# Dhole/collaborative_filtering

Measured on AMD Instinct MI355X. Metric: user-subgraph eigendecomps/sec + predicted ratings/sec, 1M users avg deg 100, higher is better.
Workload: dtype f32 (eigen) / f64 (predict)

## Files before the change

collaborative_filtering_amd/_native.py:

```python
from __future__ import annotations

import ctypes
import os
from ctypes import POINTER, c_char_p, c_double, c_float, c_int, c_int32, c_uint32, c_uint64, c_void_p

_HERE = os.path.dirname(os.path.abspath(__file__))
LIB_PATH = os.environ.get("CF_MI355X_LIB") or os.path.join(_HERE, "libcf_mi355x.so")
HOST_LIB_PATH = os.path.join(_HERE, "libcf_host.so")

CF_OK = 0
CF_EINVAL = -1
CF_ERANGE = -4
CF_SVD_MAX_NV = 256
CF_ALS_MAX_D = 64
CF_TOPN_MAX_N = 1024
CF_SIGS_OWN = 0
CF_SIGS_COMPAT = 1
CF_MAX_K = 192
CF_SPILL_MAX_K = 5000
CF_EIGEN_TRIDIAG = 0
CF_EIGEN_JACOBI = 1
CF_GRAPH_DENSE = 0
CF_GRAPH_CSR = 1
CF_FILTER_CHEBY = 0
CF_FILTER_BINOMIAL = 1

SIGNATURES = {
    "cf_version": (c_int, []),
    "cf_device_count": (c_int, []),
    "cf_create": (c_int, [c_int, POINTER(c_void_p)]),
    "cf_destroy": (None, [c_void_p]),
    "cf_release_workspaces": (c_int, [c_void_p]),
    "cf_last_error": (c_char_p, [c_void_p]),
    "cf_set_jacobi": (c_int, [c_void_p, c_float, c_int]),
    "cf_set_eigen_refine": (c_int, [c_void_p, c_int, c_float, c_float]),
    "cf_set_eigen_split": (c_int, [c_void_p, c_int]),
    "cf_debug_split_schedule": (c_int, [c_int, c_int, POINTER(c_int), POINTER(c_int), POINTER(c_int), POINTER(c_int)]),
    "cf_set_step_masks": (c_int, [c_void_p, c_int]),
    "cf_set_local_wlim": (c_int, [c_void_p, c_int]),
    "cf_debug_predict_nmax": (c_int, [c_int]),
    "cf_set_knn2_topk": (c_int, [c_void_p, c_uint32]),
    "cf_set_eigen_method": (c_int, [c_void_p, c_int]),
    "cf_debug_stats": (c_int, [c_void_p, c_int, c_void_p]),
    "cf_eigen_bucket_timing": (c_int, [c_void_p, c_int, c_void_p]),
    "cf_eigen_bucket_timing_split": (c_int, [c_void_p, c_int, c_void_p, c_void_p]),
    "cf_debug_phases": (c_int, [c_void_p, c_int, c_void_p]),
    "cf_debug_spill": (c_int, [c_void_p, c_int, c_void_p]),
    "cf_debug_tri": (c_int, [c_void_p, c_int, c_void_p]),
    "cf_item_graph_upload": (c_int, [c_void_p, c_uint32, c_void_p, c_void_p, c_void_p]),
    "cf_item_graph_upload_dense": (c_int, [c_void_p, c_uint32, c_void_p, c_int]),
    "cf_item_graph_device": (c_void_p, [c_void_p, POINTER(c_uint32)]),
    "cf_set_graph_layout": (c_int, [c_void_p, c_int]),
    "cf_graph_info": (c_int, [c_void_p, c_void_p, c_void_p, c_void_p]),
    "cf_item_cosine_edges": (c_int, [c_void_p, c_uint32, c_uint32, c_void_p, c_void_p, c_void_p, c_float, c_int, c_int,
                                     c_void_p, c_void_p, c_void_p, c_uint64, c_void_p]),
    "cf_plan_create": (c_int, [c_void_p, c_uint32, c_void_p, POINTER(c_void_p)]),
    "cf_plan_destroy": (None, [c_void_p]),
    "cf_evec_slots": (c_uint64, [c_uint32]),
    "cf_evec_offsets": (c_uint64, [c_uint32, c_void_p, c_void_p]),
    "cf_eigen_batch": (c_int, [c_void_p, c_uint32, c_void_p, c_void_p, c_void_p, c_void_p, c_void_p,
                               c_void_p, c_void_p]),
    "cf_eigen_run": (c_int, [c_void_p, c_void_p, c_void_p, c_void_p, c_void_p, c_void_p, c_void_p,
                             c_void_p, c_void_p, c_void_p]),
    "cf_predict_precomp": (c_int, [c_void_p, c_uint32, c_void_p, c_void_p, c_void_p, c_void_p, c_void_p,
                                   c_void_p, c_void_p, c_void_p, c_uint64, c_int, c_void_p, c_void_p,
                                   c_void_p]),
    "cf_predict_precomp_sel": (c_int, [c_void_p, c_uint32, c_void_p, c_void_p, c_void_p, c_void_p, c_void_p,
                                       c_void_p, c_void_p, c_void_p, c_uint64, c_int, c_void_p, c_void_p,
                                       c_void_p, c_void_p]),
# ... 169 lines not shown
```

collaborative_filtering_amd/api.py:

```python
from __future__ import annotations

from ctypes import byref, c_double, c_float, c_int, c_uint32, c_void_p
from dataclasses import dataclass

import numpy as np

from . import _native
from ._native import CF_ERANGE, CF_FILTER_BINOMIAL, CF_FILTER_CHEBY, CF_SIGS_COMPAT, CF_SIGS_OWN, NativeError, ptr


def _check(lib, ctx, rc, what):
    if rc != _native.CF_OK:
        msg = lib.cf_last_error(ctx)
        raise NativeError(f"{what} failed ({rc}): {msg.decode() if msg else ''}")


def evec_offsets(item_off: np.ndarray) -> tuple[np.ndarray, int]:
    k = np.diff(item_off.astype(np.int64))
    slots = k * np.maximum(k, 2)
    off = np.zeros(len(k), dtype=np.uint64)
    if len(k):
        off[1:] = np.cumsum(slots)[:-1]
    return off, int(slots.sum())

# ... 149 lines not shown
            self.lib.cf_destroy(self.h)
            self.h = None

    def release_workspaces(self):
        self._chk(self.lib.cf_release_workspaces(self.h), "cf_release_workspaces")

    def __enter__(self):
        return self

    def __exit__(self, *exc):
        self.close()

    def __del__(self):
        try:
            self.close()
        except Exception:
            pass

    def _chk(self, rc, what):
        _check(self.lib, self.h, rc, what)

    def set_eigen_method(self, method: str = "jacobi"):
        code = {"tridiag": _native.CF_EIGEN_TRIDIAG, "jacobi": _native.CF_EIGEN_JACOBI}[method]
        self._chk(self.lib.cf_set_eigen_method(self.h, code), "cf_set_eigen_method")

    def set_jacobi(self, tol_scale: float = 1.0, max_sweeps: int = 30):
        self._chk(self.lib.cf_set_jacobi(self.h, tol_scale, max_sweeps), "cf_set_jacobi")

    def set_eigen_refine(self, enable: bool = True, stop_rel: float = 1e-3, delta: float = 1e-2):
        self._chk(self.lib.cf_set_eigen_refine(self.h, int(enable), stop_rel, delta), "cf_set_eigen_refine")

    def set_eigen_split(self, enable=True):
        self._chk(self.lib.cf_set_eigen_split(self.h, int(enable)), "cf_set_eigen_split")

    def set_local_wlim(self, bisect: bool = True):
        self._chk(self.lib.cf_set_local_wlim(self.h, int(bisect)), "cf_set_local_wlim")

    def set_step_masks(self, enable: bool = True):
        self._chk(self.lib.cf_set_step_masks(self.h, int(enable)), "cf_set_step_masks")

    def debug_stats(self, enable: bool = True, read: bool = False):
        out = np.zeros(8, dtype=np.uint64) if read else None
        self._chk(self.lib.cf_debug_stats(self.h, int(enable), ptr(out)), "cf_debug_stats")
        if read:
            n = max(int(out[1]), 1)
            return {"sweeps_mean": int(out[0]) / n, "users": int(out[1]), "sweeps_max": int(out[2]),
                    "capped": int(out[3]), "assembly_cyc_per_user": int(out[4]) / n,
                    "jacobi_cyc_per_user": int(out[5]) / n, "epilogue_cyc_per_user": int(out[6]) / n,
                    "jacobi_cyc_per_step": int(out[5]) / max(int(out[7]), 1)}
        return None

    def eigen_bucket_timing(self, enable: bool = True, read: bool = False, sweeps: bool = False):
        out = np.zeros(13, dtype=np.float32) if read else None
        sw = np.zeros(13, dtype=np.float32) if read else None
        self._chk(self.lib.cf_eigen_bucket_timing_split(self.h, int(enable), ptr(out), ptr(sw)),
                  "cf_eigen_bucket_timing_split")
        return (out, sw) if sweeps else out

    def debug_spill(self, enable: bool = True, read: bool = False):
        out = np.zeros(8, dtype=np.uint64) if read else None
        self._chk(self.lib.cf_debug_spill(self.h, int(enable), ptr(out)), "cf_debug_spill")
        if read:
            n = max(int(out[0]), 1)
            names = ["assembly", "tridiag", "accumulate", "ql", "ql_gen"]
            r = {f"{nm}_cyc_per_user": int(out[i + 1]) / n for i, nm in enumerate(names)}
            r.update(users=int(out[0]), ql_iters_per_user=int(out[6]) / n, output_cyc_per_user=int(out[7]) / n)
# ... 790 lines not shown
```

collaborative_filtering_amd/csrc/cf_eigen.hip:

```cpp

#include "cf_eigen_common.h"

namespace {
using namespace cf_eig;

template <int EMAX, bool NARROW = false>
struct EigenGeom {
    static constexpr int NR = 16 * EMAX;
    static constexpr int NC = NARROW ? 188 : NR;
    static constexpr int E2 = NR / (2 * kGroup);
    static constexpr int LD16 = NR + ((16 - NR) % 64 + 64) % 64;
    static constexpr int LD = (NC * LD16 + 9 * NR <= 40960 - 4) ? LD16 : NR + 8;
    static constexpr int NT = (NR > 128) ? 1024 : 512;
    static constexpr int WPE = EMAX <= 5 ? 6 : 4;

    static constexpr size_t bytes() {
        return sizeof(float) * (size_t)NC * LD
               + sizeof(uint32_t) * NR
               + sizeof(float) * NR * 5
               + sizeof(int) * NR
               + sizeof(int) * 4;
    }
};
static_assert(EigenGeom<12, true>::LD % 64 == 16, "narrow bucket-12 layout must be conflict-free");
// ... 531 lines not shown
            int steps = 0;
            for (int L = 0; ((n + (1 << L) - 1) >> L) >= 2; ++L) steps += (((n + (1 << L) - 1) >> L) + 1) >> 1;
            atomicAdd(&a.stats[7], (unsigned long long)((sweep + 1) * steps));
        }
    }
}

template <int EMAX, bool NARROW = false, bool RESUME = false>
int launch_bucket_k(cf_ctx* ctx, const EigenArgs& args, uint32_t count, hipStream_t stream) {
    using G = EigenGeom<EMAX, NARROW>;
    const size_t lds = G::bytes();
    static_assert(G::bytes() <= 163840, "eigen bucket exceeds 160 KiB LDS");
    static bool configured = false;
    if (!configured) {
        CF_HIP_CHECK(ctx, hipFuncSetAttribute((const void*)eigen_kernel<EMAX, NARROW, RESUME>,
                                              hipFuncAttributeMaxDynamicSharedMemorySize, (int)lds));
        configured = true;
    }
    hipLaunchKernelGGL((eigen_kernel<EMAX, NARROW, RESUME>), dim3(count), dim3(G::NT), lds, stream, args);
    CF_HIP_CHECK(ctx, hipGetLastError());
    return CF_OK;
}

template <int EMAX, bool NARROW = false>
int launch_bucket(cf_ctx* ctx, const EigenArgs& args, uint32_t count, hipStream_t stream, uint32_t kmax = 0) {
    if constexpr (EMAX >= kSplitEmaxLow) {
        bool handled = false, finished = false;
        CF_TRY(launch_split_sweeps(ctx, args, EMAX, count, kmax, stream, &handled, &finished));
        if (handled && finished) return CF_OK;
        if (handled) {
            if (ctx->split_mid_ev) {
                CF_HIP_CHECK(ctx, hipEventRecord(ctx->split_mid_ev, stream));
                ctx->split_mid_recorded = true;
            }
            return launch_bucket_k<EMAX, NARROW, true>(ctx, args, count, stream);
        }
    }
    return launch_bucket_k<EMAX, NARROW, false>(ctx, args, count, stream);
}

int launch_bucket12_layout(cf_ctx* ctx, const EigenArgs& args, uint32_t count, uint32_t kmax, hipStream_t stream) {
    static const bool narrow_on = [] {
        const char* e = getenv("CF_EIGEN_NARROW");
        return !(e && e[0] == '0');
    }();
    if (narrow_on && kmax <= (uint32_t)EigenGeom<12, true>::NC) return launch_bucket<12, true>(ctx, args, count, stream, kmax);
    return launch_bucket<12>(ctx, args, count, stream, kmax);
}

int launch_bucket12(cf_ctx* ctx, const cf_plan* plan, const EigenArgs& args, uint32_t count, uint32_t kmax,
                    hipStream_t stream) {
    if (plan && args.mode == kUser && kmax > (uint32_t)kSplitKmax12 && count > 1) {
        auto k_at = [&](uint32_t j) {
            const uint32_t u = plan->h_order[args.first + j];
            return (uint32_t)(plan->h_item_off[u + 1] - plan->h_item_off[u]);
        };
        uint32_t lo = 0, hi = count;
        while (lo < hi) {
            const uint32_t mid = (lo + hi) / 2;
            if (k_at(mid) > (uint32_t)kSplitKmax12) lo = mid + 1;
            else hi = mid;
        }
        if (lo > 0 && lo < count) {
            CF_TRY(launch_bucket12_layout(ctx, args, lo, kmax, stream));
            EigenArgs rest = args;
            rest.first += lo;
// ... 315 lines not shown
```

collaborative_filtering_amd/csrc/cf_eigen_common.h:

```cpp
#pragma once

#include "cf_internal.h"

namespace cf_eig {

constexpr int kGroup = 8;
#ifndef CF_EIGEN_SIGROT2
#define CF_EIGEN_SIGROT2 256.0f
#endif
constexpr float kSigRot2 = CF_EIGEN_SIGROT2;

using f2 = __attribute__((ext_vector_type(2))) float;
using f4 = __attribute__((ext_vector_type(4))) float;
__device__ __forceinline__ f2 lds_ld(const f2* p) {
    return *(const volatile __attribute__((address_space(3))) f2*)(p);
}
__device__ __forceinline__ void lds_st(f2* p, f2 v) {
#if defined(CF_EIGEN_FUSED_ST) && CF_EIGEN_FUSED_ST
    *p = v;
#else
    *(volatile __attribute__((address_space(3))) f2*)(p) = v;
#endif
}

// ... 39 lines not shown
    const uint32_t* pair_user;
    const uint64_t* test_off;
    const uint32_t* test_user;
    const float* test_rating;
    float* wlim;
    const int* only_flag;
    uint64_t* cmask_out;
    uint64_t cmask_words;
    uint64_t* cmask_fp;
    uint32_t cmask_users;
    const uint8_t* solved;
    int skip_spill;
    int skip_emax_min;
};

__device__ __forceinline__ float test_rating(const EigenArgs& a, uint32_t movie, uint32_t user) {
    uint64_t lo = a.test_off[movie];
    const uint64_t end = a.test_off[movie + 1];
    uint64_t hi = end;
    while (lo < hi) {
        const uint64_t mid = (lo + hi) >> 1;
        if (a.test_user[mid] < user) lo = mid + 1;
        else hi = mid;
    }
    return (lo < end && a.test_user[lo] == user) ? a.test_rating[lo] : 0.0f;
}

constexpr int kSplitEmaxMin = 9;
constexpr int kSplitEmaxLow = 5;
constexpr int kSplitKmax12 = 180;
int launch_split_sweeps(cf_ctx* ctx, const EigenArgs& a, int emax, uint32_t count, uint32_t kmax, hipStream_t stream,
                        bool* handled, bool* finished);

}
```

collaborative_filtering_amd/csrc/cf_eigen_split.hip:

```cpp

#include <array>
#include <mutex>

#include "cf_eigen_common.h"

namespace cf_eig {
namespace {

constexpr int kMaxLev = 9;
constexpr uint32_t kNone = 0xFFFFFFFFu;
constexpr uint32_t kRoleActive = 1u << 31;
constexpr uint32_t kTrWrite = 1u << 31;
constexpr uint32_t kTrRead = 1u << 30;
constexpr int kTrFLShift = 16;

constexpr int split_ld(int nr) {
    int ld = nr;
    while (ld % 64 != 16 && ld % 64 != 48) ++ld;
    return ld;
}

constexpr int split_upc(int emax) { return emax >= 9 ? 2 : 3; }

template <int EMAX>
// ... 1020 lines not shown
        const int RBo = (NS * LD) / LDO;
        for (int i0 = 0; i0 < k; i0 += RBo) {
            const int rb = min(RBo, k - i0);
            for (int idx = tid; idx < rb * k; idx += NT) {
                const int r = idx / k, c = idx - r * k;
                tile[r * LDO + c] = hb[(size_t)(i0 + r) * k + c];
            }
            __syncthreads();
            for (int idx = tid; idx < rb * lim; idx += NT) {
                const int r = idx / lim, cc = idx - r * lim;
                float v = 0.0f;
                if (cc < k) {
                    const int jj = s_map[cc];
                    v = tile[r * LDO + jj] * s_s[jj];
                }
                hb[(size_t)(i0 + r) * lim + cc] = v;
            }
            __syncthreads();
        }
    }
    if (a.stats && tid == 0) {
        const unsigned long long t3 = __builtin_amdgcn_s_memtime();
        atomicAdd(&a.stats[0], (unsigned long long)(sweep + 1));
        atomicAdd(&a.stats[1], 1ull);
        atomicMax(&a.stats[2], (unsigned long long)(sweep + 1));
        if (sweep >= a.max_sweeps) atomicAdd(&a.stats[3], 1ull);
        atomicAdd(&a.stats[4], s_stamp[1] - s_stamp[0]);
        atomicAdd(&a.stats[5], s_stamp[2] - s_stamp[1]);
        if (FINISH) atomicAdd(&a.stats[6], t3 - s_stamp[2]);
        atomicAdd(&a.stats[7], (unsigned long long)((sweep + 1) * steps_sweep));
    }
}

template <int EMAX, bool FINISH>
int launch_split_kernel(cf_ctx* ctx, const EigenArgs& a, uint32_t count, hipStream_t stream) {
    using G = SplitGeom<EMAX>;
    static bool configured = false;
    if (!configured) {
        CF_HIP_CHECK(ctx, hipFuncSetAttribute((const void*)split_sweep_kernel<EMAX, FINISH>,
                                              hipFuncAttributeMaxDynamicSharedMemorySize, (int)G::bytes()));
        configured = true;
    }
    hipLaunchKernelGGL((split_sweep_kernel<EMAX, FINISH>), dim3(count), dim3(G::NT), G::bytes(), stream, a,
                       (const uint32_t*)ctx->d_split_sched[EMAX]);
    CF_HIP_CHECK(ctx, hipGetLastError());
    return CF_OK;
}

template <int EMAX>
int launch_emax_split(cf_ctx* ctx, const EigenArgs& a, uint32_t count, uint32_t kmax, hipStream_t stream,
                      bool* handled, bool* finished) {
    int ok_hi = 0;
    const std::vector<uint32_t>& tab = host_table<EMAX>(&ok_hi);
    if ((int)kmax > ok_hi) return CF_OK;
    if (!ctx->d_split_sched[EMAX]) {
        void* p = nullptr;
        CF_TRY(cf_malloc_evict(ctx, &p, tab.size() * sizeof(uint32_t), "split sweep schedule"));
        ctx->d_split_sched[EMAX] = static_cast<uint32_t*>(p);
        CF_HIP_CHECK(ctx, hipMemcpy(p, tab.data(), tab.size() * sizeof(uint32_t), hipMemcpyHostToDevice));
    }
    if (ctx->split_finish < 0) {
        const char* e = getenv("CF_EIGEN_SPLIT_FINISH");
        ctx->split_finish = !e ? 2 : (e[0] == '1') ? 1 : 0;
    }
    if (ctx->split_finish == 1 || (ctx->split_finish == 2 && EMAX <= 8)) {
        CF_TRY((launch_split_kernel<EMAX, true>(ctx, a, count, stream)));
// ... 1 lines not shown
    } else {
        CF_TRY((launch_split_kernel<EMAX, false>(ctx, a, count, stream)));
    }
    *handled = true;
    return CF_OK;
}

}

int launch_split_sweeps(cf_ctx* ctx, const EigenArgs& a, int emax, uint32_t count, uint32_t kmax, hipStream_t stream,
                        bool* handled, bool* finished) {
    *handled = false;
    *finished = false;
    if (a.mode != kUser || emax < kSplitEmaxLow || emax > 12 || count == 0) return CF_OK;
    if (ctx->eigen_split < 0) {
        const char* e = getenv("CF_EIGEN_SPLIT");
        ctx->eigen_split = e ? atoi(e) : 1;
    }
    const int emin = ctx->eigen_split == 1 ? kSplitEmaxMin : ctx->eigen_split;
    if (!ctx->eigen_split || emax < emin) return CF_OK;
    switch (emax) {
        case 5: return launch_emax_split<5>(ctx, a, count, kmax, stream, handled, finished);
        case 6: return launch_emax_split<6>(ctx, a, count, kmax, stream, handled, finished);
        case 7: return launch_emax_split<7>(ctx, a, count, kmax, stream, handled, finished);
        case 8: return launch_emax_split<8>(ctx, a, count, kmax, stream, handled, finished);
        case 9: return launch_emax_split<9>(ctx, a, count, kmax, stream, handled, finished);
        case 10: return launch_emax_split<10>(ctx, a, count, kmax, stream, handled, finished);
        case 11: return launch_emax_split<11>(ctx, a, count, kmax, stream, handled, finished);
        case 12: return launch_emax_split<12>(ctx, a, count, kmax, stream, handled, finished);
        default: return CF_OK;
    }
}

}

using namespace cf_eig;

extern "C" int cf_set_eigen_split(cf_ctx* ctx, int enable) {
    if (!ctx) return CF_EINVAL;
    if (enable < 0 || (enable > 1 && (enable < kSplitEmaxLow || enable > 12))) return CF_EINVAL;
    ctx->eigen_split = enable;
    return CF_OK;
}

namespace {
template <int EMAX>
void geom_of(int* ng, int* ns, int* klo, int* khi) {
    *ng = SplitGeom<EMAX>::NG;
    *ns = SplitGeom<EMAX>::NS;
    *klo = SplitGeom<EMAX>::KLO;
    *khi = SplitGeom<EMAX>::KHI;
}
}

extern "C" int cf_debug_split_schedule(int emax, int k, int* steps, int* levels, int* max_groups, int* max_slots) {
    int NG, NS, klo, khi;
    switch (emax) {
        case 5: geom_of<5>(&NG, &NS, &klo, &khi); break;
        case 6: geom_of<6>(&NG, &NS, &klo, &khi); break;
        case 7: geom_of<7>(&NG, &NS, &klo, &khi); break;
        case 8: geom_of<8>(&NG, &NS, &klo, &khi); break;
        case 9: geom_of<9>(&NG, &NS, &klo, &khi); break;
        case 10: geom_of<10>(&NG, &NS, &klo, &khi); break;
        case 11: geom_of<11>(&NG, &NS, &klo, &khi); break;
        case 12: geom_of<12>(&NG, &NS, &klo, &khi); break;
        default: return CF_ERANGE;
    }
    if (k < klo || k > khi) return CF_ERANGE;
    Schedule S;
// ... 10 lines not shown
```

collaborative_filtering_amd/csrc/cf_internal.h:

```cpp
#pragma once

#include <hip/hip_runtime.h>

#include <algorithm>
#include <cstdint>
#include <string>
#include <vector>

#include "cf_abi.h"

struct GraphRow {
    const float* dense;
    const uint32_t* col;
    const float* w;
    uint32_t len;
    __device__ __forceinline__ float operator[](uint32_t b) const {
        if (dense) return dense[b];
        uint32_t lo = 0, hi = len;
        while (lo < hi) {
            const uint32_t mid = (lo + hi) >> 1;
            if (col[mid] < b) lo = mid + 1;
            else hi = mid;
        }
        return (lo < len && col[lo] == b) ? w[lo] : 0.0f;
// ... 70 lines not shown
    void* d_tri = nullptr;
    size_t tri_bytes = 0;
    int eigen_method = CF_EIGEN_JACOBI;
    bool tri_debug = false;
    hipEvent_t knn_ev[3] = {nullptr, nullptr, nullptr};
    int knn_path = 0;
    unsigned int* d_knn_acc = nullptr;
    void* d_knn_part = nullptr;
    size_t knn_part_bytes = 0;
    uint32_t knn_chunk_users = 0;
    uint32_t knn2_topk = 0;
    int knn_chunks = 0;
    void* d_prep = nullptr;
    size_t prep_bytes = 0;
    hipEvent_t prep_ev[2] = {nullptr, nullptr};
    static constexpr int kAuxStreams = 2;
    hipStream_t aux_stream[kAuxStreams] = {};
    hipEvent_t aux_event[kAuxStreams + 1] = {};
    static constexpr int kBucketRuns = 16;
    bool bucket_timing = false;
    hipEvent_t bucket_ev[kBucketRuns][13][3] = {};
    bool bucket_recorded[kBucketRuns][13] = {};
    bool bucket_mid[kBucketRuns][13] = {};
    hipEvent_t split_mid_ev = nullptr;
    bool split_mid_recorded = false;
    int bucket_run = 0;
    hipStream_t step_stream[2] = {};
    hipEvent_t step_bucket_ev[16] = {};
    hipEvent_t step_sync_ev[4] = {};
    hipEvent_t step_time_ev[3] = {};
    uint32_t* d_split_sched[13] = {};
    int eigen_split = -1;
    int split_finish = -1;
    float filter_ms = 0.0f;
    uint64_t filter_nnz = 0;
    void* d_als = nullptr;
    size_t als_bytes = 0;
    float sgd_reduce_ms[2] = {0.0f, 0.0f};
    float svdpp_reduce_ms[3] = {0.0f, 0.0f, 0.0f};
    uint32_t topn_block = 0;
};

constexpr int kSpillBucket = -1;

struct cf_bucket {
    int emax = 0;

    uint32_t count = 0;
    uint32_t first = 0;
    uint32_t kmax = 0;
};

struct cf_tri_chunk {
    int emax;
    uint32_t first;
    uint32_t count;
    uint32_t kmax;
    uint32_t group;
};
struct cf_tri_group {
    uint32_t first;
    uint32_t count;
    uint32_t kmax;
};

struct cf_plan {
// ... 178 lines not shown
```

collaborative_filtering_amd/csrc/cf_pack.hip:

```cpp

#include <algorithm>
#include <thread>
#include <vector>

#include "cf_internal.h"

namespace {

constexpr int kScanThreads = 1024;

__global__ void __launch_bounds__(kScanThreads) pack_offsets_kernel(uint32_t n_users, const uint64_t* item_off,
                                                                    const int32_t* m, uint64_t* packed_off) {
    __shared__ uint64_t s_sum[kScanThreads];
    const uint32_t t = threadIdx.x;
    const uint32_t chunk = (n_users + kScanThreads - 1) / kScanThreads;
    const uint32_t u0 = min(n_users, t * chunk), u1 = min(n_users, u0 + chunk);
    uint64_t s = 0;
    for (uint32_t u = u0; u < u1; ++u) s += (item_off[u + 1] - item_off[u]) * (uint64_t)max(m[u], 0);
    s_sum[t] = s;
    __syncthreads();
    for (int d = 1; d < kScanThreads; d <<= 1) {
        const uint64_t v = t >= (uint32_t)d ? s_sum[t - d] : 0;
        __syncthreads();
        s_sum[t] += v;
        __syncthreads();
    }
    uint64_t run = s_sum[t] - s;
    for (uint32_t u = u0; u < u1; ++u) {
        packed_off[u] = run;
        run += (item_off[u + 1] - item_off[u]) * (uint64_t)max(m[u], 0);
    }
    if (t == kScanThreads - 1) packed_off[n_users] = s_sum[t];
}

__global__ void __launch_bounds__(256) pack_copy_kernel(uint32_t n_users, const uint64_t* item_off, const int32_t* m,
                                                        const uint64_t* evec_off, const float* evecs,
                                                        const uint64_t* packed_off, float* packed) {
    for (uint32_t u = blockIdx.x; u < n_users; u += gridDim.x) {
        const uint64_t n = (item_off[u + 1] - item_off[u]) * (uint64_t)max(m[u], 0);
        const float* src = evecs + evec_off[u];
        float* dst = packed + packed_off[u];
        const uint64_t mis_s = ((uintptr_t)src >> 2) & 3, mis_d = ((uintptr_t)dst >> 2) & 3;
        if (mis_s == mis_d) {
            const uint64_t head = min<uint64_t>(n, (4 - mis_s) & 3);
            for (uint64_t i = threadIdx.x; i < head; i += blockDim.x) dst[i] = src[i];
            const uint64_t nv = (n - head) / 4;
            const float4* s4 = reinterpret_cast<const float4*>(src + head);
            float4* d4 = reinterpret_cast<float4*>(dst + head);
            for (uint64_t i = threadIdx.x; i < nv; i += blockDim.x) d4[i] = s4[i];
            for (uint64_t i = head + nv * 4 + threadIdx.x; i < n; i += blockDim.x) dst[i] = src[i];
        } else {
            for (uint64_t i = threadIdx.x; i < n; i += blockDim.x) dst[i] = src[i];
        }
    }
}

void cost_split(uint32_t n_users, const uint64_t* item_off, int n_parts, uint32_t* split) {
    std::vector<double> cum(n_users + 1, 0.0);
    for (uint32_t u = 0; u < n_users; ++u) {
        const double k = (double)(item_off[u + 1] - item_off[u]);
        cum[u + 1] = cum[u] + k * k * k;
    }
    split[0] = 0;
    for (int p = 1; p < n_parts; ++p) {
        const double target = cum[n_users] * (double)p / (double)n_parts;
// ... 38 lines not shown
            for (uint32_t u = 0; u <= nu; ++u) off[u] = item_off[u0 + u] - e0;
            for (uint32_t u = 0; u < nu; ++u) eoff[u] = evec_off[u0 + u] - lo;
            const bool compat = sig_mode == CF_SIGS_COMPAT;
            rcs[d] = sel(ctxs[d], nu, off.data(), items + e0, ratings + e0, m + u0, evals + e0,
                                            eoff.data(), evecs + lo, compat ? sigtab : sigtab + e0,
                                            compat ? sigtab_len : ne, sig_mode, row_sel ? row_sel + e0 : nullptr,
                                            mse + e0, kk + e0, pred ? pred + e0 : nullptr);
        });
    for (auto& t : pool) t.join();
    for (int d = 0; d < n_dev; ++d)
        if (rcs[d] != CF_OK)
            return cf_set_error(root, rcs[d], "device part " + std::to_string(d) + ": " + ctxs[d]->last_error);
    (void)hipSetDevice(root->device);
    return CF_OK;
}

}

extern "C" {

int cf_cost_split(uint32_t n_users, const uint64_t* item_off, int n_parts, uint32_t* split) {
    if (!item_off || !split || n_parts <= 0) return CF_EINVAL;
    cost_split(n_users, item_off, n_parts, split);
    return CF_OK;
}

int cf_pack_eigen_run(cf_ctx* ctx, uint32_t n_users, const uint64_t* d_item_off, const int32_t* d_m,
                      const uint64_t* d_evec_off, const float* d_evecs, uint64_t* d_packed_off, float* d_packed,
                      void* stream) {
    if (!ctx || !d_item_off || !d_m || !d_packed_off) return cf_set_error(ctx, CF_EINVAL, "cf_pack_eigen_run: null");
    if (d_packed && (!d_evec_off || !d_evecs)) return cf_set_error(ctx, CF_EINVAL, "cf_pack_eigen_run: null evecs");
    CF_TRY(set_device(ctx));
    hipStream_t st = (hipStream_t)stream;
    hipLaunchKernelGGL(pack_offsets_kernel, dim3(1), dim3(kScanThreads), 0, st, n_users, d_item_off, d_m,
                       d_packed_off);
    CF_HIP_CHECK(ctx, hipGetLastError());
    if (d_packed && n_users) {
        const uint32_t blocks = std::min<uint32_t>(n_users, 65536u);
        hipLaunchKernelGGL(pack_copy_kernel, dim3(blocks), dim3(256), 0, st, n_users, d_item_off, d_m, d_evec_off,
                           d_evecs, (const uint64_t*)d_packed_off, d_packed);
        CF_HIP_CHECK(ctx, hipGetLastError());
    }
    return CF_OK;
}

struct multi_part {
    cf_ctx* ctx = nullptr;
    uint32_t u0 = 0, n = 0;
    uint64_t e0 = 0, ne = 0;
    uint64_t packed = 0;
    DevBuf off, items, eoff, m, sig, eval, evec, poff, pack;
    hipStream_t stream = nullptr;
    int rc = CF_OK;
};

static int multi_run_part(multi_part& p, const uint64_t* item_off, const uint32_t* items) {
    cf_ctx* ctx = p.ctx;
    CF_TRY(set_device(ctx));
    CF_HIP_CHECK(ctx, hipStreamCreateWithFlags(&p.stream, hipStreamNonBlocking));
    std::vector<uint64_t> off(p.n + 1), eoff(std::max<uint32_t>(p.n, 1));
    for (uint32_t u = 0; u <= p.n; ++u) off[u] = item_off[p.u0 + u] - p.e0;
    const uint64_t n_evec = cf_evec_offsets(p.n, off.data(), eoff.data());
    for (uint64_t e = 0; e < p.ne; ++e)
        if (items[p.e0 + e] >= ctx->n_items) return cf_set_error(ctx, CF_EINVAL, "item index outside the graph");
    cf_plan* plan = nullptr;
    CF_TRY(cf_plan_create(ctx, p.n, off.data(), &plan));
    int rc = dev_alloc(ctx, p.off, sizeof(uint64_t) * (p.n + 1));
    if (rc == CF_OK) rc = dev_alloc(ctx, p.items, sizeof(uint32_t) * p.ne);
    if (rc == CF_OK) rc = dev_alloc(ctx, p.eoff, sizeof(uint64_t) * eoff.size());
// ... 168 lines not shown
```

include/cf_abi.h:

```cpp
#ifndef CF_ABI_H
#define CF_ABI_H

#include <stddef.h>
#include <stdint.h>

#ifdef __cplusplus
extern "C" {
#endif

#define CF_OK 0
#define CF_EINVAL (-1)
#define CF_ENOMEM (-2)
#define CF_EHIP (-3)
#define CF_ERANGE (-4)
#define CF_ESTATE (-5)

#define CF_MAX_K 192
#define CF_SPILL_MAX_K 5000

typedef struct cf_ctx cf_ctx;
typedef struct cf_plan cf_plan;

int cf_version(void);
int cf_device_count(void);
int cf_create(int device, cf_ctx** out);
void cf_destroy(cf_ctx* ctx);
int cf_release_workspaces(cf_ctx* ctx);
const char* cf_last_error(const cf_ctx* ctx);
#define CF_EIGEN_TRIDIAG 0
#define CF_EIGEN_JACOBI 1
int cf_set_eigen_method(cf_ctx* ctx, int method);
int cf_set_jacobi(cf_ctx* ctx, float tol_scale, int max_sweeps);
int cf_set_eigen_refine(cf_ctx* ctx, int enable, float stop_rel, float delta);
int cf_set_eigen_split(cf_ctx* ctx, int enable);
int cf_debug_split_schedule(int emax, int k, int* steps, int* levels, int* max_groups, int* max_slots);
int cf_set_step_masks(cf_ctx* ctx, int enable);
int cf_set_local_wlim(cf_ctx* ctx, int bisect);
int cf_debug_stats(cf_ctx* ctx, int enable, uint64_t* out8);
int cf_debug_spill(cf_ctx* ctx, int enable, uint64_t* out8);
int cf_debug_tri(cf_ctx* ctx, int enable, uint64_t* out8);
int cf_debug_phases(cf_ctx* ctx, int enable, uint64_t* out16);
int cf_debug_predict_nmax(int lmax);
int cf_eigen_bucket_timing(cf_ctx* ctx, int enable, float* ms13);
int cf_eigen_bucket_timing_split(cf_ctx* ctx, int enable, float* ms13, float* sweeps_ms13);

#define CF_GRAPH_DENSE 0
#define CF_GRAPH_CSR 1
int cf_set_graph_layout(cf_ctx* ctx, int layout);
int cf_graph_info(const cf_ctx* ctx, int* layout, uint32_t* n_items, uint64_t* nnz);
int cf_item_graph_upload(cf_ctx* ctx, uint32_t n_items, const uint64_t* row_ptr,
                         const uint32_t* col, const float* w);
int cf_item_graph_upload_dense(cf_ctx* ctx, uint32_t n_items, const float* w_dense,
                               int on_device);
const float* cf_item_graph_device(const cf_ctx* ctx, uint32_t* n_items);

int cf_plan_create(cf_ctx* ctx, uint32_t n_users, const uint64_t* item_off, cf_plan** out);
void cf_plan_destroy(cf_plan* plan);
uint64_t cf_evec_slots(uint32_t k);
uint64_t cf_evec_offsets(uint32_t n_users, const uint64_t* item_off, uint64_t* evec_off);

int cf_eigen_batch(cf_ctx* ctx, uint32_t n_users, const uint64_t* item_off,
                   const uint32_t* items, const uint64_t* evec_off, int32_t* m_out,
                   float* sigs, float* evals, float* evecs);
int cf_eigen_run(cf_ctx* ctx, const cf_plan* plan, const uint64_t* d_item_off,
                 const uint32_t* d_items, const uint64_t* d_evec_off, int32_t* d_m,
                 float* d_sigs, float* d_evals, float* d_evecs, void* stream);

// ... 240 lines not shown
```

Before: 330,800.

## Add dedicated split-finish eigen kernel and multi-block pack offset scan

Adds a separate finish kernel for eigen buckets 9-12 after split sweeps. It does the refinement correction with MFMA, fp64 norm and sign normalisation, rank sort, limit count and transpose in a smaller-LDS workgroup sized so two fit per CU. It replaces the resumed full eigen kernel epilogue, which should improve occupancy for the tail phase. Separately, the single-block pack offset scan becomes a three-kernel multi-block decoupled scan, to remove a serial bottleneck over 1M users.

Result: no change. 332,600 (median of 6 runs) (+0.6%).

```diff
diff --git a/collaborative_filtering_amd/_native.py b/collaborative_filtering_amd/_native.py
--- a/collaborative_filtering_amd/_native.py
+++ b/collaborative_filtering_amd/_native.py
@@ -35,6 +35,7 @@
     "cf_set_jacobi": (c_int, [c_void_p, c_float, c_int]),
     "cf_set_eigen_refine": (c_int, [c_void_p, c_int, c_float, c_float]),
     "cf_set_eigen_split": (c_int, [c_void_p, c_int]),
+    "cf_set_eigen_finish": (c_int, [c_void_p, c_int]),
     "cf_debug_split_schedule": (c_int, [c_int, c_int, POINTER(c_int), POINTER(c_int), POINTER(c_int), POINTER(c_int)]),
     "cf_set_step_masks": (c_int, [c_void_p, c_int]),
     "cf_set_local_wlim": (c_int, [c_void_p, c_int]),
diff --git a/collaborative_filtering_amd/api.py b/collaborative_filtering_amd/api.py
--- a/collaborative_filtering_amd/api.py
+++ b/collaborative_filtering_amd/api.py
@@ -205,6 +205,9 @@
 
     def set_eigen_split(self, enable=True):
         self._chk(self.lib.cf_set_eigen_split(self.h, int(enable)), "cf_set_eigen_split")
+
+    def set_eigen_finish(self, mode=1):
+        self._chk(self.lib.cf_set_eigen_finish(self.h, int(mode)), "cf_set_eigen_finish")
 
     def set_local_wlim(self, bisect: bool = True):
         self._chk(self.lib.cf_set_local_wlim(self.h, int(bisect)), "cf_set_local_wlim")
diff --git a/collaborative_filtering_amd/csrc/cf_eigen.hip b/collaborative_filtering_amd/csrc/cf_eigen.hip
--- a/collaborative_filtering_amd/csrc/cf_eigen.hip
+++ b/collaborative_filtering_amd/csrc/cf_eigen.hip
@@ -587,6 +587,11 @@
             if (ctx->split_mid_ev) {
                 CF_HIP_CHECK(ctx, hipEventRecord(ctx->split_mid_ev, stream));
                 ctx->split_mid_recorded = true;
+            }
+            if constexpr (EMAX >= kSplitEmaxMin) {
+                bool launched = false;
+                CF_TRY(launch_split_finish(ctx, args, EMAX, count, stream, &launched));
+                if (launched) return CF_OK;
             }
             return launch_bucket_k<EMAX, NARROW, true>(ctx, args, count, stream);
         }
diff --git a/collaborative_filtering_amd/csrc/cf_eigen_common.h b/collaborative_filtering_amd/csrc/cf_eigen_common.h
--- a/collaborative_filtering_amd/csrc/cf_eigen_common.h
+++ b/collaborative_filtering_amd/csrc/cf_eigen_common.h
@@ -95,4 +95,6 @@
 int launch_split_sweeps(cf_ctx* ctx, const EigenArgs& a, int emax, uint32_t count, uint32_t kmax, hipStream_t stream,
                         bool* handled, bool* finished);
 
+int launch_split_finish(cf_ctx* ctx, const EigenArgs& a, int emax, uint32_t count, hipStream_t stream, bool* launched);
+
 }
diff --git a/collaborative_filtering_amd/csrc/cf_eigen_split.hip b/collaborative_filtering_amd/csrc/cf_eigen_split.hip
--- a/collaborative_filtering_amd/csrc/cf_eigen_split.hip
+++ b/collaborative_filtering_amd/csrc/cf_eigen_split.hip
@@ -1076,6 +1076,380 @@
     }
 }
 
+template <int EMAX>
+struct FinishGeom {
+    using S = SplitGeom<EMAX>;
+    static constexpr int NR = S::NR, KLO = S::KLO, KHI = S::KHI;
+    static constexpr int NW = 4, NT = 64 * NW, NG = NT / kGroup;
+    static constexpr int TJ = (EMAX + NW - 1) / NW;
+    static constexpr int CPG = (KHI + NG - 1) / NG;
+    static constexpr int SMALL = 4 * NR * 4 + 16;
+    static constexpr int STATIC = 256;
+    static constexpr int AREA = ((81920 - STATIC - SMALL) / 4) & ~3;
+    static constexpr int RB1x = ((AREA / KHI - 4) / 16) * 16;
+    static constexpr int RB1 = RB1x < NR ? RB1x : NR, LDR1 = RB1 + 4;
+    static constexpr int RB3 = 32, LDR3 = RB3 + 4;
+    static constexpr int DOFF = (KHI * LDR3 + 3) & ~3;
+    static constexpr int TB = 32, TBW = 2 * TB * (TB + 1);
+    static constexpr size_t bytes() { return (size_t)AREA * 4 + SMALL; }
+    static_assert(EMAX >= 9 && EMAX <= 12, "buckets 9-12");
+    static_assert(KLO > 16 * (EMAX - 1), "every k of the bucket has EMAX column tiles");
+    static_assert(KHI <= NT, "a thread per eigenvalue in the lim count");
+    static_assert(RB1 >= 16 && RB1 % 16 == 0 && NR * LDR1 <= AREA, "F row block (NR columns: unguarded reads)");
+    static_assert(NR * LDR3 <= AREA, "update row block (NR columns: unguarded reads)");
+    static_assert(RB3 % 16 == 0 && LDR3 % 8 == 4 && DOFF + 4 * CPG * NT <= AREA, "update row block, fp64 partials");
+    static_assert(NW * TBW <= AREA, "flip blocks");
+    static_assert(16 * (KHI + 1) <= AREA && NR <= AREA, "output row block, sigs");
+    static_assert((bytes() + STATIC) * 2 <= 163840, "two finish workgroups share a CU's LDS");
+};
+
+template <int EMAX>
+__global__ __launch_bounds__(FinishGeom<EMAX>::NT, 2) void split_finish_kernel(EigenArgs a) {
+    using G = FinishGeom<EMAX>;
+    constexpr int NR = G::NR, NW = G::NW, NT = G::NT, NG = G::NG, TJ = G::TJ, CPG = G::CPG;
+    constexpr int RB1 = G::RB1, LDR1 = G::LDR1, RB3 = G::RB3, LDR3 = G::LDR3;
+    extern __shared__ float smem[];
+    float* tile = smem;
+    float* s_mu = tile + G::AREA;
+    float* s_dev = s_mu + NR;
+    float* s_s = s_dev + NR;
+    int* s_perm = reinterpret_cast<int*>(s_s + NR);
+
+    const int tid = threadIdx.x;
+    const int wave = __builtin_amdgcn_readfirstlane(tid >> 6);
+    auto fresh = [](int x) {
+        asm volatile("" : "+v"(x));
+        return x;
+    };
+    const unsigned long long t0 = (a.stats && tid == 0) ? __builtin_amdgcn_s_memtime() : 0ull;
+    if (a.only_flag && !a.only_flag[blockIdx.x]) return;
+    const uint32_t u = a.order[a.first + blockIdx.x];
+    const uint64_t base = a.item_off[u];
+    const int k = (int)(a.item_off[u + 1] - base);
+    if (k < G::KLO || k > G::KHI) return;
+    float* hb = a.evecs + a.evec_off[u];
+    const uint32_t kk1 = (uint32_t)(k * k - 1);
+    const bool refine = a.refine != 0;
+    static_assert(TJ <= 4, "per-tile scalars travel in an f4");
+    struct Tiles {
+        int m16, kq;
+        int jc[TJ], jcs[TJ];
+        bool jv[TJ];
+    };
+    auto tiles_of = [&](int t) {
+        Tiles T;
+        T.m16 = t & 15;
+        T.kq = (t & 63) >> 4;
+#pragma unroll
+        for (int jt = 0; jt < TJ; ++jt) {
+            T.jc[jt] = (wave + NW * jt) * 16 + T.m16;
+            T.jv[jt] = T.jc[jt] < k;
+            T.jcs[jt] = T.jv[jt] ? T.jc[jt] : 0;
+        }
+        return T;
+    };
+    for (int j = tid; j < k; j += NT) s_dev[j] = a.evals[base + j];
+
+    f4 kv[TJ][EMAX];
+    if (refine) {
+        const Tiles T = tiles_of(fresh(tid));
+        const int m16 = T.m16, kq = T.kq;
+#pragma unroll
+        for (int jt = 0; jt < TJ; ++jt)
+#pragma unroll
+            for (int I = 0; I < EMAX; ++I) kv[jt][I] = f4{0.f, 0.f, 0.f, 0.f};
+        f2 nacc[CPG];
+#pragma unroll
+        for (int i = 0; i < CPG; ++i) nacc[i] = f2{0.f, 0.f};
+        for (int R0 = 0; R0 < k; R0 += RB1) {
+            __syncthreads();
+#pragma unroll 4
+            for (int idx = fresh(tid); idx < k * RB1; idx += NT) {
+                const int c = idx / RB1, r = idx - c * RB1;
+                const float v = hb[min((uint32_t)(c * k + R0 + r), kk1)];
+                tile[c * LDR1 + r] = (R0 + r < k) ? v : 0.0f;
+            }
+            __syncthreads();
+            const int nc16 = (min(RB1, k - R0) + 15) >> 4;
+            const int g = fresh(tid) / kGroup, lig = fresh(tid) % kGroup;
+#pragma unroll
+            for (int i = 0; i < CPG; ++i) {
+                const int c = g + NG * i;
+                if (c < k) {
+                    const f2* bc = reinterpret_cast<const f2*>(tile + c * LDR1) + lig;
+                    for (int e = 0; e < nc16; ++e) {
+                        const f2 x = bc[kGroup * e];
+                        nacc[i] = __builtin_elementwise_fma(x, x, nacc[i]);
+                    }
+                }
+            }
+            for (int c = 0; c < nc16; ++c) {
+                f4 y[TJ];
+#pragma unroll
+                for (int jt = 0; jt < TJ; ++jt) {
+                    const f4 y0 = *reinterpret_cast<const f4*>(tile + T.jcs[jt] * LDR1 + 16 * c + 4 * kq);
+                    y[jt] = T.jv[jt] ? y0 : f4{0.f, 0.f, 0.f, 0.f};
+                }
+                auto ldx = [&](int I) {
+                    return *reinterpret_cast<const f4*>(tile + (I * 16 + m16) * LDR1 + 16 * c + 4 * kq);
+                };
+                f4 xn = ldx(0);
+#pragma unroll
+                for (int I = 0; I < EMAX; ++I) {
+                    const f4 x = (I < EMAX - 1 || I * 16 + m16 < k) ? xn : f4{0.f, 0.f, 0.f, 0.f};
+                    if (I + 1 < EMAX) xn = ldx(I + 1);
+                    __builtin_amdgcn_sched_barrier(0);
+#pragma unroll
+                    for (int t = 0; t < 4; ++t)
+#pragma unroll
+                        for (int jt = 0; jt < TJ; ++jt)
+                            kv[jt][I] = __builtin_amdgcn_mfma_f32_16x16x4f32(x[t], y[jt][t], kv[jt][I], 0, 0, 0);
+                    __builtin_amdgcn_sched_barrier(0);
+                }
+            }
+        }
+        const int g = fresh(tid) / kGroup, lig = fresh(tid) % kGroup;
+#pragma unroll
+        for (int i = 0; i < CPG; ++i) {
+            const int c = g + NG * i;
+            const float nc = pair_sum(nacc[i].x + nacc[i].y);
+            if (c < k && lig == 0) s_mu[c] = nc / (1.0f + s_dev[c]);
+        }
+        __syncthreads();
+        const float dlt = a.refine_delta;
+        f4 muj2, muj, ksq;
+#pragma unroll
+        for (int jt = 0; jt < TJ; ++jt) {
+            muj2[jt] = T.jv[jt] ? s_mu[T.jcs[jt]] : 1.0f;
+            muj[jt] = sqrtf(muj2[jt]);
+            ksq[jt] = 0.0f;
+        }
+#pragma unroll
+        for (int I = 0; I < EMAX; ++I) {
+#pragma unroll
+            for (int r = 0; r < 4; ++r) {
+                const int i = I * 16 + 4 * kq + r;
+                const float mui2 = s_mu[I < EMAX - 1 ? i : min(i, k - 1)];
+                const float mui = sqrtf(mui2);
+#pragma unroll
+                for (int jt = 0; jt < TJ; ++jt) {
+                    float kvv = 0.0f;
+                    if (T.jv[jt] && (I < EMAX - 1 || i < k) && i != T.jc[jt] && fabsf(mui - muj[jt]) > dlt) kvv = kv[jt][I][r] / (mui2 - muj2[jt]);
+                    kv[jt][I][r] = -kvv;
+                    ksq[jt] = fmaf(kvv, kvv, ksq[jt]);
+                }
+            }
+            __builtin_amdgcn_sched_barrier(0);
+        }
+#pragma unroll
+        for (int jt = 0; jt < TJ; ++jt) {
+            float q = ksq[jt];
+            q += __shfl_xor(q, 16);
+            q += __shfl_xor(q, 32);
+            if (kq == 0 && T.jv[jt]) s_dev[T.jc[jt]] += q;
+        }
+    }
+
+    double* const s_dd0 = reinterpret_cast<double*>(tile + G::DOFF);
+#pragma unroll
+    for (int i = 0; i < 2 * CPG; ++i) s_dd0[i * NT + tid] = 0.0;
+    for (int R0 = 0; R0 < k; R0 += RB3) {
+        __syncthreads();
+#pragma unroll 4
+        for (int idx = fresh(tid); idx < k * RB3; idx += NT) {
+            const int c = idx / RB3, r = idx - c * RB3;
+            const float v = hb[min((uint32_t)(c * k + R0 + r), kk1)];
+            tile[c * LDR3 + r] = (R0 + r < k) ? v : 0.0f;
+        }
+        __syncthreads();
+        if (refine) {
+            const Tiles T = tiles_of(fresh(tid));
+            const int m16 = T.m16, kq = T.kq;
+            f4 out[TJ][RB3 / 16];
+#pragma unroll
+            for (int jt = 0; jt < TJ; ++jt)
+#pragma unroll
+                for (int q = 0; q < RB3 / 16; ++q) {
+                    const f4 o0 = *reinterpret_cast<const f4*>(tile + T.jcs[jt] * LDR3 + 16 * q + 4 * kq);
+                    out[jt][q] = T.jv[jt] ? o0 : f4{0.f, 0.f, 0.f, 0.f};
+                }
+            constexpr int NQ = RB3 / 16;
+            auto lda = [&](int I, float* av) {
+#pragma unroll
+                for (int t = 0; t < 4; ++t)
+#pragma unroll
+                    for (int q = 0; q < NQ; ++q) av[t * NQ + q] = tile[(I * 16 + 4 * kq + t) * LDR3 + 16 * q + m16];
+            };
+            float an[4 * NQ];
+            lda(0, an);
+#pragma unroll
+            for (int I = 0; I < EMAX; ++I) {
+                float av[4 * NQ];
+#pragma unroll
+                for (int t = 0; t < 4; ++t)
+#pragma unroll
+                    for (int q = 0; q < NQ; ++q) av[t * NQ + q] = (I < EMAX - 1 || I * 16 + 4 * kq + t < k) ? an[t * NQ + q] : 0.0f;
+                if (I + 1 < EMAX) lda(I + 1, an);
+                __builtin_amdgcn_sched_barrier(0);
+#pragma unroll
+                for (int t = 0; t < 4; ++t)
+#pragma unroll
+                    for (int q = 0; q < NQ; ++q)
+                        if (R0 + 16 * q < NR)
+#pragma unroll
+                            for (int jt = 0; jt < TJ; ++jt)
+                                out[jt][q] = __builtin_amdgcn_mfma_f32_16x16x4f32(av[t * NQ + q], kv[jt][I][t], out[jt][q], 0, 0, 0);
+                __builtin_amdgcn_sched_barrier(0);
+            }
+            __syncthreads();
+#pragma unroll
+            for (int jt = 0; jt < TJ; ++jt)
+                if (T.jv[jt])
+#pragma unroll
+                    for (int q = 0; q < RB3 / 16; ++q)
+                        if (R0 + 16 * q < NR) *reinterpret_cast<f4*>(tile + T.jc[jt] * LDR3 + 16 * q + 4 * kq) = out[jt][q];
+            __syncthreads();
+#pragma unroll 4
+            for (int idx = fresh(tid); idx < k * RB3; idx += NT) {
+                const int c = idx / RB3, r = idx - c * RB3;
+                if (R0 + r < k) hb[c * k + R0 + r] = tile[c * LDR3 + r];
+            }
+        }
+        const int nc16 = (min(RB3, k - R0) + 15) >> 4;
+        const int tq = fresh(tid), g = tq / kGroup, lig = tq % kGroup;
+        double* s_dd = s_dd0 + tq;
+#pragma unroll
+        for (int i = 0; i < CPG; ++i) {
+            const int c = g + NG * i;
+            if (c < k) {
+                const f2* bc = reinterpret_cast<const f2*>(tile + c * LDR3) + lig;
+                double acc = s_dd[2 * i * NT], sum = s_dd[(2 * i + 1) * NT];
+                for (int e = 0; e < nc16; ++e) {
+                    const f2 x = bc[kGroup * e];
+                    acc = fma((double)x.x, (double)x.x, acc);
+                    acc = fma((double)x.y, (double)x.y, acc);
+                    sum += (double)x.x;
+                    sum += (double)x.y;
+                }
+                s_dd[2 * i * NT] = acc;
+                s_dd[(2 * i + 1) * NT] = sum;
+            }
+        }
+    }
+    const int g = tid / kGroup, lig = tid % kGroup;
+    const double* s_dd = s_dd0 + tid;
+#pragma unroll
+    for (int i = 0; i < CPG; ++i) {
+        const int c = g + NG * i;
+        double acc = s_dd[2 * i * NT], sum = s_dd[(2 * i + 1) * NT];
+#pragma unroll
+        for (int o = 1; o < kGroup; o <<= 1) {
+            acc += __shfl_xor(acc, o);
+            sum += __shfl_xor(sum, o);
+        }
+        if (c < k && lig == 0) {
+            const double nrm = sqrt(acc);
+            s_mu[c] = (float)(nrm / sqrt(1.0 + (double)s_dev[c]));
+            s_s[c] = (float)((sum < 0.0 ? -1.0 : 1.0) / nrm);
+        }
+    }
+    __syncthreads();
+    for (int j = tid; j < k; j += NT) {
+        const float mj = s_mu[j];
+        int rank = 0;
+        for (int i = 0; i < k; ++i) {
+            const float mi = s_mu[i];
+            rank += (mi < mj) || (mi == mj && i < j);
+        }
+        s_perm[rank] = j;
+    }
+    float* s_sig = tile;
+    for (int i = tid; i < k; i += NT) s_sig[i] = a.sigs[base + i];
+    __syncthreads();
+    float smm = 0.0f;
+    for (int i = 0; i < k; ++i) smm = fmaxf(smm, s_sig[i]);
+    const bool below = tid < k && !((double)(s_mu[tid] - 1.0f) > (double)smm);
+    int lim = __syncthreads_count(below);
+    if (lim < 2) lim = 2;
+    if (tid == 0) a.m_out[u] = lim;
+    for (int r = tid; r < k; r += NT) a.evals[base + r] = r < lim ? s_mu[s_perm[r]] - 1.0f : 0.0f;
+
+    {
+        constexpr int TB = G::TB;
+        const int nbk = (k + TB - 1) / TB;
+        const int nunits = nbk * (nbk + 1) / 2;
+        float* tx = tile + wave * G::TBW;
+        float* ty = tx + TB * (TB + 1);
+        const int q = tid & (TB - 1), ph = (tid & 63) >> 5;
+        for (int u0 = 0; u0 < nunits; u0 += NW) {
+            const int unit = u0 + wave;
+            int bp = 0, rem = unit;
+            while (bp < nbk && rem >= nbk - bp) rem -= nbk - bp++;
+            const bool live = unit < nunits;
+            const int P0 = bp * TB, Q0 = (bp + rem) * TB;
+            __syncthreads();
+            if (live) {
+                float x[TB / 2], y[TB / 2];
+#pragma unroll
+                for (int it = 0; it < TB / 2; ++it) {
+                    const int p = 2 * it + ph;
+                    x[it] = hb[min((uint32_t)((P0 + p) * k + Q0 + q), kk1)];
+                    y[it] = hb[min((uint32_t)((Q0 + p) * k + P0 + q), kk1)];
+                }
+#pragma unroll
+                for (int it = 0; it < TB / 2; ++it) {
+                    const int p = 2 * it + ph;
+                    tx[p * (TB + 1) + q] = x[it];
+                    ty[p * (TB + 1) + q] = y[it];
+                }
+            }
+            __syncthreads();
+            if (live) {
+#pragma unroll
+                for (int it = 0; it < TB / 2; ++it) {
+                    const int p = 2 * it + ph;
+                    if (P0 + p < k && Q0 + q < k) hb[(P0 + p) * k + Q0 + q] = ty[q * (TB + 1) + p];
+                    if (Q0 + p < k && P0 + q < k) hb[(Q0 + p) * k + P0 + q] = tx[q * (TB + 1) + p];
+                }
+            }
+        }
+    }
+    {
+        const int LDO = k + 1;
+        const int RBo = G::AREA / LDO;
+        for (int i0 = 0; i0 < k; i0 += RBo) {
+            const int rb = min(RBo, k - i0);
+            __syncthreads();
+#pragma unroll 4
+            for (int idx = tid; idx < rb * k; idx += NT) {
+                const int r = idx / k, c = idx - r * k;
+                tile[r * LDO + c] = hb[(size_t)(i0 + r) * k + c];
+            }
+            __syncthreads();
+            for (int idx = tid; idx < rb * lim; idx += NT) {
+                const int r = idx / lim, cc = idx - r * lim;
+                const int jj = s_perm[cc];
+                hb[(size_t)(i0 + r) * lim + cc] = tile[r * LDO + jj] * s_s[jj];
+            }
+        }
+    }
+    if (a.stats && tid == 0) atomicAdd(&a.stats[6], __builtin_amdgcn_s_memtime() - t0);
+}
+
+template <int EMAX>
+int launch_finish_kernel(cf_ctx* ctx, const EigenArgs& a, uint32_t count, hipStream_t stream) {
+    using G = FinishGeom<EMAX>;
+    static bool configured = false;
+    if (!configured) {
+        CF_HIP_CHECK(ctx, hipFuncSetAttribute((const void*)split_finish_kernel<EMAX>,
+                                              hipFuncAttributeMaxDynamicSharedMemorySize, (int)G::bytes()));
+        configured = true;
+    }
+    hipLaunchKernelGGL((split_finish_kernel<EMAX>), dim3(count), dim3(G::NT), G::bytes(), stream, a);
+    CF_HIP_CHECK(ctx, hipGetLastError());
+    return CF_OK;
+}
+
 template <int EMAX, bool FINISH>
 int launch_split_kernel(cf_ctx* ctx, const EigenArgs& a, uint32_t count, hipStream_t stream) {
     using G = SplitGeom<EMAX>;
@@ -1143,9 +1517,34 @@
     }
 }
 
+int launch_split_finish(cf_ctx* ctx, const EigenArgs& a, int emax, uint32_t count, hipStream_t stream, bool* launched) {
+    *launched = false;
+    if (ctx->eigen_finish < 0) {
+        const char* e = getenv("CF_EIGEN_FINISH");
+        ctx->eigen_finish = e ? (atoi(e) != 0) : 1;
+    }
+    if (!ctx->eigen_finish || a.mode != kUser || count == 0) return CF_OK;
+    switch (emax) {
+        case 9: CF_TRY(launch_finish_kernel<9>(ctx, a, count, stream)); break;
+        case 10: CF_TRY(launch_finish_kernel<10>(ctx, a, count, stream)); break;
+        case 11: CF_TRY(launch_finish_kernel<11>(ctx, a, count, stream)); break;
+        case 12: CF_TRY(launch_finish_kernel<12>(ctx, a, count, stream)); break;
+        default: return CF_OK;
+    }
+    *launched = true;
+    return CF_OK;
+}
+
 }
 
 using namespace cf_eig;
+
+extern "C" int cf_set_eigen_finish(cf_ctx* ctx, int mode) {
+    if (!ctx) return CF_EINVAL;
+    if (mode != 0 && mode != 1) return CF_EINVAL;
+    ctx->eigen_finish = mode;
+    return CF_OK;
+}
 
 extern "C" int cf_set_eigen_split(cf_ctx* ctx, int enable) {
     if (!ctx) return CF_EINVAL;
diff --git a/collaborative_filtering_amd/csrc/cf_internal.h b/collaborative_filtering_amd/csrc/cf_internal.h
--- a/collaborative_filtering_amd/csrc/cf_internal.h
+++ b/collaborative_filtering_amd/csrc/cf_internal.h
@@ -126,6 +126,7 @@
     uint32_t* d_split_sched[13] = {};
     int eigen_split = -1;
     int split_finish = -1;
+    int eigen_finish = -1;
     float filter_ms = 0.0f;
     uint64_t filter_nnz = 0;
     void* d_als = nullptr;
diff --git a/collaborative_filtering_amd/csrc/cf_pack.hip b/collaborative_filtering_amd/csrc/cf_pack.hip
--- a/collaborative_filtering_amd/csrc/cf_pack.hip
+++ b/collaborative_filtering_amd/csrc/cf_pack.hip
@@ -7,30 +7,81 @@
 
 namespace {
 
-constexpr int kScanThreads = 1024;
+constexpr int kScanThreads = 256;
+constexpr int kScanPer = 4;
+constexpr int kScanTile = kScanThreads * kScanPer;
+
+__device__ __forceinline__ uint64_t pack_len(uint64_t u, uint32_t n_users, const uint64_t* item_off,
+                                             const int32_t* m) {
+    return u < n_users ? (item_off[u + 1] - item_off[u]) * (uint64_t)max(m[u], 0) : 0;
+}
+
+__device__ __forceinline__ uint64_t block_scan_incl(uint64_t v, uint64_t* s_wave, uint64_t* total) {
+    constexpr int NW = kScanThreads / 64;
+    const int lane = threadIdx.x & 63, wave = threadIdx.x >> 6;
+#pragma unroll
+    for (int d = 1; d < 64; d <<= 1) {
+        const uint64_t o = __shfl_up(v, d);
+        if (lane >= d) v += o;
+    }
+    __syncthreads();
+    if (lane == 63) s_wave[wave] = v;
+    __syncthreads();
+    uint64_t before = 0, all = 0;
+#pragma unroll
+    for (int w = 0; w < NW; ++w) {
+        const uint64_t x = s_wave[w];
+        if (w < wave) before += x;
+        all += x;
+    }
+    *total = all;
+    return v + before;
+}
+
+__global__ void __launch_bounds__(kScanThreads) pack_tile_sums_kernel(uint32_t n_users, const uint64_t* item_off,
+                                                                      const int32_t* m, uint64_t* packed_off) {
+    __shared__ uint64_t s_wave[kScanThreads / 64];
+    const uint64_t u0 = (uint64_t)blockIdx.x * kScanTile + threadIdx.x;
+    uint64_t s = 0;
+#pragma unroll
+    for (int q = 0; q < kScanPer; ++q) {
+        const uint64_t u = u0 + (uint64_t)q * kScanThreads;
+        s += pack_len(u, n_users, item_off, m);
+    }
+    uint64_t total;
+    (void)block_scan_incl(s, s_wave, &total);
+    if (threadIdx.x == 0) packed_off[(uint64_t)blockIdx.x * kScanTile] = total;
+}
+
+__global__ void __launch_bounds__(kScanThreads) pack_tile_scan_kernel(uint32_t n_users, uint32_t n_tiles,
+                                                                      uint64_t* packed_off) {
+    __shared__ uint64_t s_wave[kScanThreads / 64];
+    uint64_t run = 0;
+    for (uint32_t t0 = 0; t0 < n_tiles; t0 += kScanThreads) {
+        const uint32_t t = t0 + threadIdx.x;
+        const uint64_t v = t < n_tiles ? packed_off[(uint64_t)t * kScanTile] : 0;
+        uint64_t total;
+        const uint64_t incl = block_scan_incl(v, s_wave, &total);
+        if (t < n_tiles) packed_off[(uint64_t)t * kScanTile] = run + incl - v;
+        run += total;
+    }
+    if (threadIdx.x == 0) packed_off[n_users] = run;
+}
 
 __global__ void __launch_bounds__(kScanThreads) pack_offsets_kernel(uint32_t n_users, const uint64_t* item_off,
                                                                     const int32_t* m, uint64_t* packed_off) {
-    __shared__ uint64_t s_sum[kScanThreads];
-    const uint32_t t = threadIdx.x;
-    const uint32_t chunk = (n_users + kScanThreads - 1) / kScanThreads;
-    const uint32_t u0 = min(n_users, t * chunk), u1 = min(n_users, u0 + chunk);
-    uint64_t s = 0;
-    for (uint32_t u = u0; u < u1; ++u) s += (item_off[u + 1] - item_off[u]) * (uint64_t)max(m[u], 0);
-    s_sum[t] = s;
-    __syncthreads();
-    for (int d = 1; d < kScanThreads; d <<= 1) {
-        const uint64_t v = t >= (uint32_t)d ? s_sum[t - d] : 0;
-        __syncthreads();
-        s_sum[t] += v;
-        __syncthreads();
-    }
-    uint64_t run = s_sum[t] - s;
-    for (uint32_t u = u0; u < u1; ++u) {
-        packed_off[u] = run;
-        run += (item_off[u + 1] - item_off[u]) * (uint64_t)max(m[u], 0);
-    }
-    if (t == kScanThreads - 1) packed_off[n_users] = s_sum[t];
+    __shared__ uint64_t s_wave[kScanThreads / 64];
+    const uint64_t u0 = (uint64_t)blockIdx.x * kScanTile + threadIdx.x;
+    uint64_t run = packed_off[(uint64_t)blockIdx.x * kScanTile];
+#pragma unroll
+    for (int q = 0; q < kScanPer; ++q) {
+        const uint64_t u = u0 + (uint64_t)q * kScanThreads;
+        const uint64_t v = pack_len(u, n_users, item_off, m);
+        uint64_t total;
+        const uint64_t incl = block_scan_incl(v, s_wave, &total);
+        if (u < n_users) packed_off[u] = run + incl - v;
+        run += total;
+    }
 }
 
 __global__ void __launch_bounds__(256) pack_copy_kernel(uint32_t n_users, const uint64_t* item_off, const int32_t* m,
@@ -135,9 +186,19 @@
     if (d_packed && (!d_evec_off || !d_evecs)) return cf_set_error(ctx, CF_EINVAL, "cf_pack_eigen_run: null evecs");
     CF_TRY(set_device(ctx));
     hipStream_t st = (hipStream_t)stream;
-    hipLaunchKernelGGL(pack_offsets_kernel, dim3(1), dim3(kScanThreads), 0, st, n_users, d_item_off, d_m,
-                       d_packed_off);
+    const uint32_t n_tiles = (uint32_t)(((uint64_t)n_users + kScanTile - 1) / kScanTile);
+    if (n_tiles) {
+        hipLaunchKernelGGL(pack_tile_sums_kernel, dim3(n_tiles), dim3(kScanThreads), 0, st, n_users, d_item_off, d_m,
+                           d_packed_off);
+        CF_HIP_CHECK(ctx, hipGetLastError());
+    }
+    hipLaunchKernelGGL(pack_tile_scan_kernel, dim3(1), dim3(kScanThreads), 0, st, n_users, n_tiles, d_packed_off);
     CF_HIP_CHECK(ctx, hipGetLastError());
+    if (n_tiles) {
+        hipLaunchKernelGGL(pack_offsets_kernel, dim3(n_tiles), dim3(kScanThreads), 0, st, n_users, d_item_off, d_m,
+                           d_packed_off);
+        CF_HIP_CHECK(ctx, hipGetLastError());
+    }
     if (d_packed && n_users) {
         const uint32_t blocks = std::min<uint32_t>(n_users, 65536u);
         hipLaunchKernelGGL(pack_copy_kernel, dim3(blocks), dim3(256), 0, st, n_users, d_item_off, d_m, d_evec_off,
diff --git a/include/cf_abi.h b/include/cf_abi.h
--- a/include/cf_abi.h
+++ b/include/cf_abi.h
@@ -33,6 +33,7 @@
 int cf_set_jacobi(cf_ctx* ctx, float tol_scale, int max_sweeps);
 int cf_set_eigen_refine(cf_ctx* ctx, int enable, float stop_rel, float delta);
 int cf_set_eigen_split(cf_ctx* ctx, int enable);
+int cf_set_eigen_finish(cf_ctx* ctx, int mode);
 int cf_debug_split_schedule(int emax, int k, int* steps, int* levels, int* max_groups, int* max_slots);
 int cf_set_step_masks(cf_ctx* ctx, int enable);
 int cf_set_local_wlim(cf_ctx* ctx, int bisect);
```
